# facebookresearch/r3m

Measured on AMD Instinct MI355X. Metric: encoder frames/sec (fwd+bwd) ResNet-50 224^2 bs=256/GPU, higher is better.
Workload: dtype f32

## Files before the change

r3m_amd/csrc/common.h:

```cpp
#pragma once
#include <hip/hip_runtime.h>
#include <stdint.h>
#include <stddef.h>

#ifdef R3M_PROBES
#include <cstdlib>
#define R3M_ENV_INT(name, dflt) ([]() -> int { static const int v_ = []() { const char* e_ = getenv(name); return e_ ? atoi(e_) : (dflt); }(); return v_; }())
#define R3M_PROBE(p) ((p).debug)
#else
#define R3M_ENV_INT(name, dflt) (dflt)
#define R3M_PROBE(p) 0
#endif

namespace r3m {

typedef float f32x4 __attribute__((ext_vector_type(4)));
typedef float f32x16 __attribute__((ext_vector_type(16)));

void set_last_error(const char* fmt, ...);
int  check_launch(const char* what);

#define R3M_REQUIRE(cond, ...)                  \
  do {                                          \
    if (!(cond)) {                              \
// ... 38 lines not shown
  const float* bn_scale;
  const float* bn_shift;
  const float* bn_mean;
  int N, Hi, Wi, Ci;
  int Hg, Wg;
  int Ho, Wo, Nc;
  int is;
  int os, ooy, oox;
  int M;
  int T;
  int ntaps;
  int flags;
  int simple_rows;
  int debug;
  int dtype;
  unsigned* tile_ctr;
  signed char dy[MAX_TAPS];
  signed char dx[MAX_TAPS];
  unsigned char wt[MAX_TAPS];
  int tap[MAX_TAPS];
};

struct WgradParams {
  const float* dY;
  const float* X;
  float* out;
  int N, Hi, Wi, Ci;
  int Ho, Wo, Co;
  int KH, KW, stride, pad;
  int M;
  int simple_rows;
  int dtype;
  int rows_per_split;
  int tilesN;
  int gx;
  int xcd;
  int debug;
};

int debug_occupancy(int* out4);
int launch_gather_gemm(const GatherGemmParams& p, hipStream_t s);
double gather_gemm_alg_bytes(const GatherGemmParams& p, int elem_bytes);
bool gather_gemm_fuses_affine(const GatherGemmParams& p);
int gather_gemm_grid_m(int M, int Nc);
void gg_set_tile_counters(unsigned* ctr8, int sets = 1);
int gg_set_dynamic_tiles(int on);
void gg_route_record_begin(int* out, int cap);
int gg_route_record_end();
struct WtEntry { long long w_off, wt_off; int Co, T, Ci, pad_; };
int launch_transpose_w_all(const float* params, void* wt, const WtEntry* tab, const int* tile0, int n, int tiles, int dt, hipStream_t s);
int launch_transpose_w(const float* W, float* Wt, int Co, int T, int Ci, hipStream_t s);

bool pw_gemm_eligible(const GatherGemmParams& p);
int pw_gemm_form(const GatherGemmParams& p);
int launch_pw_gemm(const GatherGemmParams& p, hipStream_t s);

enum : int {
  WG_TAPS_SIMPLE = 40,
  WG_TAPS_GATHER = 41,
  WG_ROWS        = 42,
  WG_WINDOW      = 43,
  WG16_TAPS      = 50,
  WG16_ROWS      = 51,
  WG16_ALL_TAPS  = 52,
};
struct WgradPlan {
  int route, tile, bk;
  int fast;
  int split, rows_per_split;
  int tilesN, gx;
  int lds_bytes;
  int xcd, debug;
};
WgradPlan wgrad_plan(const WgradParams& p);
int launch_wgrad(const WgradParams& p, const WgradPlan& r, hipStream_t s);
int launch_wgrad_reduce(const float* partial, float* dW, long long n, int splitK, int accumulate, hipStream_t s);
int wgrad_debug_occupancy(int* out);
bool wgrad_rowwin_eligible(const WgradParams& p);
int wgrad_rowwin_lds_bytes(int tile);
int launch_wgrad_rowwin(const WgradParams& p, const WgradPlan& r, hipStream_t s);
bool wgrad_halo_eligible(const WgradParams& p);
int wgrad_halo_lds_bytes(int W);
int launch_wgrad_bf16(const WgradParams& p, const WgradPlan& r, hipStream_t s);

int launch_gather_gemm_bf16(const GatherGemmParams& p, hipStream_t s);
bool gg16_route_builds(int route, int flags);
int gg16_route(const GatherGemmParams& p);
int launch_convert_bf16(const float* src, void* dst, long long n, hipStream_t s);
int launch_transpose_w_bf16(const float* W, void* Wt, int Co, int T, int Ci, hipStream_t s);

bool row16_eligible(const GatherGemmParams& p);
int launch_conv3x3_row_bf16(const GatherGemmParams& p, hipStream_t s);
int row16_set_mode(int mode);

#ifdef R3M_PROBES
int pw16_form(const GatherGemmParams& p);
int launch_pw16(const GatherGemmParams& p, hipStream_t s);
int pw16_set_mode(int mode);
#else
static inline int pw16_form(const GatherGemmParams&) { return 0; }
static inline int launch_pw16(const GatherGemmParams&, hipStream_t) { return 1; }
static inline int pw16_set_mode(int) { return -1; }
#endif

struct FrameSource;
int launch_stem_prep(const float* x_nchw, float* xn, int F, hipStream_t s);
// ... 117 lines not shown
```

r3m_amd/csrc/conv.hip:

```cpp
#include "common.h"
#include "conv_dev.h"
#include <utility>

namespace r3m {

__device__ __attribute__((aligned(128))) float g_zero_line[2048 + 64];


template <int EPI>
__global__ __launch_bounds__(256) void gather_gemm_glds_kernel(const GatherGemmParams p) {
  constexpr int BM = 128, BN = 128, WM = 2, WN = 2, TM = 2, TN = 2;
  constexpr int STAGE = (BM + BN) * 32;
  __shared__ __attribute__((aligned(128))) float smem[2 * STAGE];

  const int tid = threadIdx.x;
  const int lane = tid & 63;
  const int wave = tid >> 6;
  const int wm = wave / WN, wn = wave % WN;
  const int gridN = (p.Nc + BN - 1) / BN;
  const int lid = xcd_remap(blockIdx.x, gridDim.x);
  const int mt = lid / gridN, nt = lid % gridN;
  const int m0 = mt * BM, n0 = nt * BN;

  const int srow = lane >> 3;
// ... 763 lines not shown

static inline bool gg_wide(int Nc) { return (Nc % 128) == 0; }

int gather_gemm_grid_m(int M, int Nc) { return gg_wide(Nc) ? ceil_div(M, 128) : ceil_div(M, 256); }

static int gg_use_glds() {
  const int v = R3M_ENV_INT("R3M_GG_GLDS", 2);
  return v;
}

#define GG_EPI_SWITCH(LAUNCH)                                                       \
  switch (p.flags) {                                                                \
    case 0: LAUNCH(0); break;                                                       \
    case EPI_STATS: LAUNCH(EPI_STATS); break;                                       \
    case EPI_ACCUM: LAUNCH(EPI_ACCUM); break;                                       \
    case EPI_MASKED_ADD: LAUNCH(EPI_MASKED_ADD); break;                             \
    case EPI_BIAS: LAUNCH(EPI_BIAS); break;                                         \
    case EPI_RELU: LAUNCH(EPI_RELU); break;                                         \
    case EPI_BIAS | EPI_RELU: LAUNCH(EPI_BIAS | EPI_RELU); break;                   \
    case EPI_MASK_OUT: LAUNCH(EPI_MASK_OUT); break;                                 \
    case EPI_BNRED: LAUNCH(EPI_BNRED); break;                                       \
    case EPI_BNRED | EPI_MASKED_ADD: LAUNCH(EPI_BNRED | EPI_MASKED_ADD); break;     \
    default:                                                                        \
      set_last_error("gather_gemm: unsupported epilogue flag combination %d", p.flags); \
      return 1;                                                                     \
  }

double gather_gemm_alg_bytes(const GatherGemmParams& p, int elem) {
  const double in = p.simple_rows ? (double)p.M * p.Ci : (double)p.N * p.Hi * p.Wi * p.Ci;
  const double out = (double)p.M * p.Nc;
  double b = elem * (in + out + (double)p.Nc * p.ntaps * p.Ci);
  if (p.flags & EPI_ACCUM) b += elem * out;
  if (p.flags & EPI_MASKED_ADD) b += elem * out + out / 8.0;
  if (p.flags & EPI_MASK_OUT) b += elem * out;
  if (p.flags & EPI_BNRED) b += elem * out + (p.bn_bits ? out / 8.0 : 0.0) + 8.0 * bnred_partial_rows(p.M) * p.Nc;
  return b;
}

static thread_local unsigned* t_tile_ctr = nullptr;
static thread_local int t_tile_ctr_sets = 0;
static int g_dynamic_tiles = 1;
void gg_set_tile_counters(unsigned* ctr8, int sets) {
  t_tile_ctr = g_dynamic_tiles ? ctr8 : nullptr;
  t_tile_ctr_sets = t_tile_ctr ? sets : 0;
}
int gg_set_dynamic_tiles(int on) { const int old = g_dynamic_tiles; g_dynamic_tiles = on ? 1 : 0; return old; }

enum : int { GG_ROUTE_WIN = 1, GG_ROUTE_PW = 10 , GG_ROUTE_K16 = 20,
             GG_ROUTE_GLDS2 = 21, GG_ROUTE_OTHER = 22, GG_ROUTE_BF16 = 30 };
static int gg_route(const GatherGemmParams& p) {
  if (p.dtype == DT_BF16) return GG_ROUTE_BF16;
  const bool glds2 = gg_use_glds() == 2 && ((p.Ci >> 5) & 1) == 0 && p.Ci <= 2048;
  if (gg_wide(p.Nc)) {
    if (R3M_ENV_INT("R3M_GG_WIN", 1) && conv3x3_win_eligible(p, 28)) return GG_ROUTE_WIN;
    if (R3M_ENV_INT("R3M_GG_PW", 1) && pw_gemm_eligible(p)) return GG_ROUTE_PW + pw_gemm_form(p);
    const int k16_mode = R3M_ENV_INT("R3M_GG_K16", 1);
    if ((p.Ci & 31) == 0 && (k16_mode == 2 || (k16_mode == 1 && p.ntaps == 1 && p.Ci <= 256 && p.Nc >= 2 * p.Ci))) return GG_ROUTE_K16;
    return glds2 ? GG_ROUTE_GLDS2 : GG_ROUTE_OTHER;
  }
  if (R3M_ENV_INT("R3M_GG_PW", 1) && pw_gemm_eligible(p)) return GG_ROUTE_PW + pw_gemm_form(p);
  return glds2 ? GG_ROUTE_GLDS2 : GG_ROUTE_OTHER;
}

static void gg_prepare(GatherGemmParams& p) {
  for (int t = 0; t < p.ntaps; ++t)
    p.tap[t] = (int)((unsigned)(unsigned char)p.dy[t] | ((unsigned)(unsigned char)p.dx[t] << 8) | ((unsigned)p.wt[t] << 16));
  p.debug = R3M_ENV_INT("R3M_GG_DEBUG", 0);
}

bool gather_gemm_fuses_affine(const GatherGemmParams& p_in) {
  GatherGemmParams p = p_in;
  gg_prepare(p);
  if (p.dtype == DT_BF16) return (p.Nc & 7) == 0 && (p.Ci & 63) == 0 && gg16_route_builds(gg16_route(p), p.flags);
  const int r = gg_route(p);
  if (r == GG_ROUTE_WIN) return p.flags == (EPI_AFFINE | EPI_RELU) || p.flags == (EPI_AFFINE | EPI_ACCUM | EPI_RELU);
  return r > GG_ROUTE_PW && r < GG_ROUTE_K16;
}
static thread_local int* t_route_out = nullptr;
static thread_local int t_route_n = 0, t_route_cap = 0;
void gg_route_record_begin(int* out, int cap) { t_route_out = out; t_route_n = 0; t_route_cap = cap; }
int gg_route_record_end() { const int n = t_route_n; t_route_out = nullptr; t_route_n = t_route_cap = 0; return n; }
static int gg_route_record(int route) {
  if (t_route_n < t_route_cap) t_route_out[t_route_n] = route;
  ++t_route_n;
  return 0;
}

enum : int { GG_OTHER_GLDS, GG_OTHER_NARROW, GG_OTHER_REG };
static int gg_other_kernel(bool wide) {
  if (!wide) return GG_OTHER_NARROW;
#ifdef R3M_PROBES
  if (!gg_use_glds()) return GG_OTHER_REG;
#endif
  return GG_OTHER_GLDS;
}

int launch_gather_gemm(const GatherGemmParams& p_in, hipStream_t s) {
  GatherGemmParams p = p_in;
  p.tile_ctr = t_tile_ctr;
  if (t_tile_ctr && --t_tile_ctr_sets > 0) t_tile_ctr += 8;
  else { t_tile_ctr = nullptr; t_tile_ctr_sets = 0; }
  R3M_REQUIRE(p.ntaps >= 0 && p.ntaps <= MAX_TAPS, "gather_gemm: ntaps=%d", p.ntaps);
  R3M_REQUIRE(p.M > 0 && p.Nc > 0, "gather_gemm: empty problem M=%d Nc=%d", p.M, p.Nc);
  gg_prepare(p);
  if (p.dtype == DT_BF16) {
    if (t_route_out) return gg_route_record(gg16_route(p));
// ... 149 lines not shown
```

r3m_amd/csrc/conv_pw.hip:

```cpp
#include "common.h"
#include "conv_dev.h"

namespace r3m {

constexpr int PW_RSRC_FLAGS = 0x00020000;

__device__ __forceinline__ float pw_ld(const void* base, int bytes, unsigned voff, int soff) {
#if defined(__HIP_DEVICE_COMPILE__)
  return __builtin_bit_cast(float, __builtin_amdgcn_raw_buffer_load_b32(
                                       __builtin_amdgcn_make_buffer_rsrc(const_cast<void*>(base), 0, bytes, PW_RSRC_FLAGS), voff, soff, 0));
#else
  return 0.f;
#endif
}
__device__ __forceinline__ unsigned pw_ldu(const void* base, int bytes, unsigned voff, int soff) {
#if defined(__HIP_DEVICE_COMPILE__)
  return __builtin_amdgcn_raw_buffer_load_b32(__builtin_amdgcn_make_buffer_rsrc(const_cast<void*>(base), 0, bytes, PW_RSRC_FLAGS), voff, soff, 0);
#else
  return 0u;
#endif
}
typedef unsigned pw_u32x4 __attribute__((ext_vector_type(4)));
__device__ __forceinline__ f32x4 pw_ld4(const void* base, int bytes, unsigned voff, int soff) {
#if defined(__HIP_DEVICE_COMPILE__)
  return __builtin_bit_cast(f32x4, __builtin_amdgcn_raw_buffer_load_b128(
                                       __builtin_amdgcn_make_buffer_rsrc(const_cast<void*>(base), 0, bytes, PW_RSRC_FLAGS), voff, soff, 0));
#else
  return f32x4{0.f, 0.f, 0.f, 0.f};
#endif
}
#ifndef PW_ST_MOD
#define PW_ST_MOD ""
#endif
__device__ __forceinline__ void pw_st4(void* base, int bytes, unsigned voff, int soff, f32x4 v) {
#if defined(__HIP_DEVICE_COMPILE__)
  const unsigned long long a = reinterpret_cast<unsigned long long>(base);
  const pw_u32x4 rsrc = {(unsigned)a, (unsigned)(a >> 32) & 0xFFFFu, (unsigned)bytes, (unsigned)PW_RSRC_FLAGS};
  asm volatile("buffer_store_dwordx4 %0, %1, %2, %3 offen" PW_ST_MOD "\n\ts_nop 3" ::"v"(v), "v"(voff), "s"(rsrc), "s"(soff) : "memory");
#endif
}
typedef unsigned pw_u32x2 __attribute__((ext_vector_type(2)));
__device__ __forceinline__ pw_u32x2 pw_ld2(const void* base, int bytes, unsigned voff) {
#if defined(__HIP_DEVICE_COMPILE__)
  return __builtin_amdgcn_raw_buffer_load_b64(__builtin_amdgcn_make_buffer_rsrc(const_cast<void*>(base), 0, bytes, PW_RSRC_FLAGS), voff, 0, 0);
#else
  return pw_u32x2{0u, 0u};
#endif
}
__device__ __forceinline__ void pw_st(void* base, int bytes, unsigned voff, int soff, float v) {
#if defined(__HIP_DEVICE_COMPILE__)
  __builtin_amdgcn_raw_buffer_store_b32(__builtin_bit_cast(unsigned, v), __builtin_amdgcn_make_buffer_rsrc(base, 0, bytes, PW_RSRC_FLAGS), voff,
                                        soff, 0);
#endif
}

__device__ __forceinline__ const float* pw_uniform_ptr(const float* q) {
  const unsigned long long v = reinterpret_cast<unsigned long long>(q);
  const unsigned lo = __builtin_amdgcn_readfirstlane((unsigned)v), hi = __builtin_amdgcn_readfirstlane((unsigned)(v >> 32));
  return reinterpret_cast<const float*>(((unsigned long long)hi << 32) | lo);
}

template <int BM, int BN, int WM, int WN, int EPI, bool YBITS = false, bool GATHER = false, bool OSTR = false, bool BURST = false>
__global__ __launch_bounds__(WM * WN * 64, WM * WN == 4 ? 2 : 1) void pw_gemm_kernel(const GatherGemmParams p, const int tiles, const int gridN) {
  constexpr int NW = WM * WN, TN = BN / WN / 32;
  static_assert(BM / WM == 64 && (TN == 1 || TN == 2) && (NW == 4 || NW == 8), "wave tile is 64 rows x 32 TN columns");
  constexpr int STAGE = (BM + BN) * 32;
  constexpr int AJ = BM / (8 * NW), BJ = BN / (8 * NW), NP = AJ + BJ;
  static_assert(AJ >= 1 && BJ >= 1 && (NP <= 8 || BURST), "a wave stages whole DMA instructions, at most one per odd MFMA slot (burst: any number)");
  constexpr int NST = 8 * TN;
  constexpr int SR = BN >= 128 ? 128 : 256, R = BM / SR;
  static_assert(R >= 1 && WM % R == 0 && (WM / R) * 64 == SR, "wave rows nest in statistics rows");
  extern __shared__ __attribute__((aligned(128))) float smem[];

  const int tid = threadIdx.x, lane = tid & 63;
  const int wave_s = __builtin_amdgcn_readfirstlane(tid >> 6);
  const int wm = wave_s / WN, wn = wave_s % WN;
  const int W = gridDim.x;
  const int K = p.Ci, Nc = p.Nc, Kb = K * 4;
  const int lrow = lane & 31, lh = lane >> 5;

  unsigned voffA[AJ], voffB[BJ];
  const int KbB = (GATHER ? p.T : 1) * Kb;
  {
    const int srow = lane >> 3, pslot = lane & 7;
#pragma unroll
    for (int j = 0; j < AJ; ++j) {
      const int r = wave_s * (BM / NW) + j * 8 + srow;
      voffA[j] = (unsigned)(r * Kb + ((pslot ^ ((r >> 1) & 7)) << 4));
    }
#pragma unroll
    for (int j = 0; j < BJ; ++j) {
      const int r = wave_s * (BN / NW) + j * 8 + srow;
      voffB[j] = (unsigned)(r * KbB + ((pslot ^ ((r >> 1) & 7)) << 4));
    }
  }
  const float* dA = p.A;
  const float* dB = p.B;
  int dAbytes = 0, dsA = 0, dsB = 0;
  auto dma_piece = [&](auto stg_c, auto pc_c) __attribute__((always_inline)) {
    constexpr int STG = decltype(stg_c)::value, pc = decltype(pc_c)::value;
    if (R3M_PROBE(p) & 8) return;
    if constexpr (pc < AJ)
      buf_dma16_uniform(dA, dAbytes, smem + STG * STAGE + wave_s * (BM / NW) * 32 + pc * 8 * 32, voffA[pc], dsA);
    else
      buf_dma16_uniform(dB, BN * KbB, smem + STG * STAGE + BM * 32 + wave_s * (BN / NW) * 32 + (pc - AJ) * 8 * 32, voffB[pc - AJ], dsB);
  };
  auto dma_all = [&](auto stg_c) __attribute__((always_inline)) {
    static_for<NP>([&](auto pc_c) __attribute__((always_inline)) { dma_piece(stg_c, pc_c); });
  };
  unsigned poff[GATHER ? AJ : 1], iyx[GATHER ? AJ : 1];
  int tap_soffB = 0;
  auto aim_tile = [&](int tmt_, int tnt_) __attribute__((always_inline)) {
    const int tmt = __builtin_amdgcn_readfirstlane(tmt_), tnt = __builtin_amdgcn_readfirstlane(tnt_);
    dB = p.B + (long long)tnt * BN * (KbB / 4);
    if constexpr (!GATHER) {
      dA = p.A + (long long)tmt * BM * K;
      dAbytes = min(BM, p.M - tmt * BM) * Kb;
    } else {
      const int hw = p.Hg * p.Wg;
      const int m0t = tmt * BM;
      const int nf = __builtin_amdgcn_readfirstlane(m0t / hw);
      const long long frame = (long long)p.Hi * p.Wi * K;
      dA = pw_uniform_ptr(p.A + nf * frame);
      const long long rest = (long long)(p.N - nf) * frame * 4;
      dAbytes = __builtin_amdgcn_readfirstlane(rest < (long long)BUF_OOB ? (int)rest : (int)BUF_OOB);
      const int srow = lane >> 3, pslot = lane & 7;
      const int r0 = wave_s * (BM / NW) + srow;
      int m = m0t + r0;
      int n = m / hw;
      int rem = m - n * hw;
      int gy = rem / p.Wg;
      int gx = rem - gy * p.Wg;
#pragma unroll
      for (int j = 0; j < AJ; ++j) {
        const int r = r0 + j * 8;
        const int iy0 = gy * p.is, ix0 = gx * p.is;
        poff[j] = (unsigned)(((((n - nf) * p.Hi + iy0) * p.Wi + ix0) * K) * 4 + ((pslot ^ ((r >> 1) & 7)) << 4));
        iyx[j] = m < p.M ? (unsigned)((iy0 << 16) | ix0) : 0x40004000u;
        m += 8;
        gx += 8;
#pragma unroll
        for (int w = 0; w < 2; ++w) {
          const bool c = gx >= p.Wg;
          gx -= c ? p.Wg : 0;
          gy += c ? 1 : 0;
        }
#pragma unroll
        for (int w = 0; w < 2; ++w) {
          const bool c = gy >= p.Hg;
          gy -= c ? p.Hg : 0;
          n += c ? 1 : 0;
        }
      }
    }
  };
  auto set_tap = [&](int t) __attribute__((always_inline)) {
    if constexpr (GATHER) {
      const int pack = __builtin_amdgcn_readfirstlane(p.tap[t]);
      const int dy = (pack << 24) >> 24, dx = (pack << 16) >> 24, wt = pack >> 16;
      const int delta = (dy * p.Wi + dx) * Kb;
      tap_soffB = wt * Kb;
#pragma unroll
      for (int j = 0; j < AJ; ++j) {
        const unsigned iy = (iyx[j] >> 16) + (unsigned)dy, ix = (iyx[j] & 0xFFFFu) + (unsigned)dx;
        voffA[j] = (iy < (unsigned)p.Hi && ix < (unsigned)p.Wi) ? poff[j] + (unsigned)delta : BUF_OOB;
      }
    }
  };
  auto aim_step = [&](int chunk) __attribute__((always_inline)) {
    dsA = __builtin_amdgcn_readfirstlane(chunk * 128);
    dsB = __builtin_amdgcn_readfirstlane(tap_soffB + chunk * 128);
  };

  const float* fa[4];
  const float* fb[4];
  {
    const int xr = (lrow >> 1) & 7;
#pragma unroll
    for (int g = 0; g < 4; ++g) {
      const int go = ((2 * g + lh) ^ xr) * 4;
      fa[g] = smem + (wm * 64 + lrow) * 32 + go;
      fb[g] = smem + BM * 32 + (wn * TN * 32 + lrow) * 32 + go;
    }
  }
  f32x16 acc[2][TN];

  constexpr bool MADD = (EPI & EPI_MASKED_ADD) != 0, BNR = (EPI & EPI_BNRED) != 0, ACC = (EPI & EPI_ACCUM) != 0;
  constexpr bool AFF = (EPI & EPI_AFFINE) != 0, RELU = (EPI & EPI_RELU) != 0;
  static_assert(!(AFF && (BNR || MADD)) && (!RELU || AFF), "EPI_AFFINE / EPI_RELU: forward epilogues");
  constexpr bool PRE = MADD || BNR || ACC;
  static_assert(!(MADD && ACC), "one added tensor");
  constexpr int LPR = 8 * TN, RPS = 64 / LPR;
  const int srow = lane / LPR, scol = (lane % LPR) * 4;
  const unsigned vo4 = (unsigned)(((wm * 64 + srow) * Nc + wn * TN * 32 + scol) * 4);
  const int Nw = Nc >> 5;
  const unsigned vow = (unsigned)(((wm * 64 + lane) * Nw + wn * TN) * 4);
  f32x4 pg[PRE ? NST : 1], py[PRE ? NST : 1];
  typedef unsigned u32x2 __attribute__((ext_vector_type(2)));
  u32x2 pgm = {0u, 0u}, pym = {0u, 0u};
  const float* t_gb = nullptr;
  const float* t_yb = nullptr;
  const unsigned* t_gbits = nullptr;
  const unsigned* t_ybits = nullptr;
  int t_obytes = 0, t_bbytes = 0;
  static_assert(!OSTR || (GATHER && !MADD && !YBITS), "strided output rows: gather form, no mask words");
  unsigned orows[OSTR ? NST : 1];
  long long t_eo = 0;
  auto pre_tile = [&](int tmt, int tnt) __attribute__((always_inline)) {
    if constexpr (OSTR) {
      const int m0 = tmt * BM, n0 = tnt * BN;
      const int hw = p.Hg * p.Wg;
      const int nf = __builtin_amdgcn_readfirstlane(m0 / hw);
      const long long oframe = (long long)p.Ho * p.Wo * Nc;
      t_eo = nf * oframe + n0;
      const long long rest = ((long long)(p.N - nf) * oframe - n0) * 4;
      t_obytes = __builtin_amdgcn_readfirstlane(rest < (long long)BUF_OOB ? (int)rest : (int)BUF_OOB);
      const int m = m0 + wm * 64 + lane;
      const int n = m / hw;
      const int rem = m - n * hw;
      const int gy = rem / p.Wg, gx = rem - gy * p.Wg;
      const unsigned mine = m < p.M ? (unsigned)(((((n - nf) * p.Ho + gy * p.os + p.ooy) * p.Wo + gx * p.os + p.oox) * Nc) * 4) : BUF_OOB;
#pragma unroll
      for (int st = 0; st < NST; ++st)
        orows[st] = (unsigned)__builtin_amdgcn_ds_bpermute(4 * (st * RPS + srow), (int)mine) + (unsigned)((wn * TN * 32 + scol) * 4);
      if constexpr (ACC) t_gb = p.out + t_eo;
      if constexpr (BNR) t_yb = p.bn_y + t_eo;
    } else if constexpr (PRE) {
      const int m0 = tmt * BM, n0 = tnt * BN;
      const int rows_valid = min(BM, p.M - m0);
      const long long eo0 = (long long)m0 * Nc + n0;
      t_obytes = ((rows_valid - 1) * Nc + BN) * 4;
      t_bbytes = ((rows_valid - 1) * Nw + BN / 32) * 4;
      if constexpr (MADD) { t_gb = p.add0 + eo0; t_gbits = p.addbits + (eo0 >> 5); }
      if constexpr (ACC) t_gb = p.out + eo0;
      if constexpr (BNR) { t_yb = p.bn_y + eo0; t_ybits = YBITS ? p.bn_bits + (eo0 >> 5) : nullptr; }
    }
  };
  auto pre_piece = [&](auto pc_c) __attribute__((always_inline)) {
    if constexpr (PRE) {
      constexpr int pc = decltype(pc_c)::value;
      if (R3M_PROBE(p) & 16) return;
      int ncb = Nc * 4;
      asm volatile("" : "+s"(ncb));
      const int so = OSTR ? 0 : (pc * RPS) * ncb;
      const unsigned vo = OSTR ? orows[OSTR ? pc : 0] : vo4;
      if constexpr (MADD || ACC) pg[pc] = pw_ld4(t_gb, t_obytes, vo, so);
      if constexpr (BNR) py[pc] = pw_ld4(t_yb, t_obytes, vo, so);
      if constexpr (pc == 0) {
        if constexpr (MADD) {
          if constexpr (TN == 2) pgm = pw_ld2(t_gbits, t_bbytes, vow);
          else pgm[0] = pw_ldu(t_gbits, t_bbytes, vow, 0);
        }
        if constexpr (BNR && YBITS) {
          if constexpr (TN == 2) pym = pw_ld2(t_ybits, t_bbytes, vow);
          else pym[0] = pw_ldu(t_ybits, t_bbytes, vow, 0);
        }
      }
    }
  };

  auto kstep = [&](auto stgm_c, auto first_c, auto dma_c, auto pf_c, bool do_dma, bool do_pf) __attribute__((always_inline)) {
    constexpr int STG_M = decltype(stgm_c)::value, PF = decltype(pf_c)::value;
    constexpr bool FIRST = decltype(first_c)::value, DMA = decltype(dma_c)::value;
    using SD = std::integral_constant<int, STG_M ^ 1>;
    constexpr int FB = ((MADD && BNR) || (GATHER && BNR && AJ > 4)) ? 1 : 2;
    f32x4 af[FB][2], bf[FB][TN];
    auto frag_load = [&](auto g_c) __attribute__((always_inline)) {
      constexpr int g = decltype(g_c)::value;
#pragma unroll
      for (int t = 0; t < 2; ++t) af[g % FB][t] = *reinterpret_cast<const f32x4*>(fa[g] + STG_M * STAGE + t * 32 * 32);
#pragma unroll
      for (int t = 0; t < TN; ++t) bf[g % FB][t] = *reinterpret_cast<const f32x4*>(fb[g] + STG_M * STAGE + t * 32 * 32);
    };
    if constexpr (FB == 2) frag_load(std::integral_constant<int, 0>{});
    static_for<4>([&](auto g_c) __attribute__((always_inline)) {
      constexpr int g = decltype(g_c)::value;
      if constexpr (FB == 1) frag_load(g_c);
      if constexpr (FB == 2 && g < 3) frag_load(std::integral_constant<int, g + 1>{});
      const f32x4(&a)[2] = af[g % FB];
      const f32x4(&b)[TN] = bf[g % FB];
      static_for<4>([&](auto j_c) __attribute__((always_inline)) {
        constexpr int j = decltype(j_c)::value;
#pragma unroll
        for (int tm = 0; tm < 2; ++tm)
#pragma unroll
          for (int tn = 0; tn < TN; ++tn) {
            if constexpr (FIRST && g == 0 && j == 0) {
              const f32x16 z = {0.f, 0.f, 0.f, 0.f, 0.f, 0.f, 0.f, 0.f, 0.f, 0.f, 0.f, 0.f, 0.f, 0.f, 0.f, 0.f};
              acc[tm][tn] = __builtin_amdgcn_mfma_f32_32x32x2f32(a[tm][j], b[tn][j], z, 0, 0, 0);
            } else {
              acc[tm][tn] = __builtin_amdgcn_mfma_f32_32x32x2f32(a[tm][j], b[tn][j], acc[tm][tn], 0, 0, 0);
            }
          }
        if constexpr (PRE && PF != 0) {
          constexpr int slot = g * 4 + j;
// ... 9 lines not shown
          constexpr int slot = g * 4 + j;
          constexpr bool fire = (slot & 1) == 1 && (slot >> 1) < NP;
          constexpr int piece = slot >> 1;
          if constexpr (fire) {
            if (do_dma) {
              __builtin_amdgcn_sched_barrier(0);
              dma_piece(SD{}, std::integral_constant<int, piece>{});
              __builtin_amdgcn_sched_barrier(0);
            }
          }
        }
      });
    });
  };

  constexpr int CW = TN * 32;
  float* const slabs = smem + 2 * STAGE;
  float* slab = slabs + wave_s * (8 * CW);
  float* slab_w = slab + 4 * lh * CW + lrow;
  const float* slab_r = slab + srow * CW + scol;
  const int bp0 = 4 * srow;
  const bool hiw = TN == 2 && (lane & 8) != 0;
  const int nsh = (lane & 7) * 4;
  auto mask_nibble = [&](const u32x2& words, int st) __attribute__((always_inline)) -> unsigned {
    const unsigned w0 = (unsigned)__builtin_amdgcn_ds_bpermute(bp0 + st * RPS * 4, (int)words[0]);
    unsigned w = w0;
    if constexpr (TN == 2) {
      const unsigned w1 = (unsigned)__builtin_amdgcn_ds_bpermute(bp0 + st * RPS * 4, (int)words[1]);
      w = hiw ? w1 : w0;
    }
    return (w >> nsh) & 15u;
  };
  auto epilogue1 = [&](int emt, int ent) __attribute__((always_inline)) {
    const int m0 = emt * BM, n0 = ent * BN;
    if (R3M_PROBE(p) & 4) return;
    float st_s[TN], st_ss[TN];
    if ((EPI & EPI_STATS) != 0 && !(R3M_PROBE(p) & 2)) {
#pragma unroll
      for (int tn = 0; tn < TN; ++tn) {
        float s = 0.f, ss = 0.f;
#pragma unroll
        for (int tm = 0; tm < 2; ++tm)
#pragma unroll
          for (int r = 0; r < 16; ++r) {
            const float v = acc[tm][tn][r];
            s += v;
            ss = fmaf(v, v, ss);
          }
        st_s[tn] = s + __shfl_xor(s, 32);
        st_ss[tn] = ss + __shfl_xor(ss, 32);
      }
    }
    const int rows_valid = min(BM, p.M - m0);
    const long long eo0 = (long long)m0 * Nc + n0;
    const int obytes = OSTR ? t_obytes : ((rows_valid - 1) * Nc + BN) * 4;
    float* ob = p.out + (OSTR ? t_eo : eo0);
    f32x4 s1 = {0.f, 0.f, 0.f, 0.f}, s2 = s1, mu = s1, sc = s1, sh = s1;
    if constexpr (BNR) {
      const int col = n0 + wn * CW + scol;
      mu = *reinterpret_cast<const f32x4*>(p.bn_mean + col);
      if constexpr (!YBITS) {
        sc = *reinterpret_cast<const f32x4*>(p.bn_scale + col);
        sh = *reinterpret_cast<const f32x4*>(p.bn_shift + col);
      }
    }
    if constexpr (AFF) {
      const int col = n0 + wn * CW + scol;
      sc = *reinterpret_cast<const f32x4*>(p.bn_scale + col);
      sh = *reinterpret_cast<const f32x4*>(p.bn_shift + col);
    }
    static_for<8>([&](auto c_c) __attribute__((always_inline)) {
      constexpr int c = decltype(c_c)::value;
      constexpr int tm = c >> 2, q = c & 3;
#pragma unroll
      for (int tn = 0; tn < TN; ++tn)
#pragma unroll
        for (int e = 0; e < 4; ++e) slab_w[e * CW + tn * 32] = acc[tm][tn][4 * q + e];
      __builtin_amdgcn_wave_barrier();
      int ncb = Nc * 4;
      asm volatile("" : "+s"(ncb));
#pragma unroll
      for (int i = 0; i < TN; ++i) {
        const int st = c * TN + i;
        f32x4 v = *reinterpret_cast<const f32x4*>(slab_r + i * RPS * CW);
        if constexpr (AFF) {
#pragma unroll
          for (int e = 0; e < 4; ++e) v[e] = fmaf(v[e], sc[e], sh[e]);
        }
        if constexpr (ACC) v += pg[st];
        if constexpr (RELU) {
#pragma unroll
          for (int e = 0; e < 4; ++e) v[e] = fmaxf(v[e], 0.f);
        }
        if constexpr (MADD) {
          const unsigned nb = mask_nibble(pgm, st);
#pragma unroll
          for (int e = 0; e < 4; ++e) v[e] += ((nb >> e) & 1u) ? pg[st][e] : 0.f;
        }
        if (!(R3M_PROBE(p) & 1)) pw_st4(ob, obytes, OSTR ? orows[OSTR ? st : 0] : vo4, OSTR ? 0 : (st * RPS) * ncb, v);
        if constexpr (BNR) {
          const f32x4 y = py[st];
          unsigned nb = 0u;
          if constexpr (YBITS) nb = mask_nibble(pym, st);
#pragma unroll
          for (int e = 0; e < 4; ++e) {
            const bool on = YBITS ? (((nb >> e) & 1u) != 0u) : (fmaf(y[e], sc[e], sh[e]) > 0.f);
            const float gg = on ? v[e] : 0.f;
            s1[e] += gg;
            s2[e] = fmaf(gg, y[e] - mu[e], s2[e]);
          }
        }
      }
      __builtin_amdgcn_wave_barrier();
    });
    if ((EPI & EPI_STATS) != 0 && !(R3M_PROBE(p) & 2)) {
      if (lane < 32) {
#pragma unroll
        for (int tn = 0; tn < TN; ++tn) {
          slab[tn * 32 + lane] = st_s[tn];
          slab[CW + tn * 32 + lane] = st_ss[tn];
        }
      }
    }
    if constexpr (BNR) {
      const int g0 = m0 + wm * 64;
#pragma unroll
      for (int e = 0; e < 4; ++e)
#pragma unroll
        for (int o = LPR; o < 64; o <<= 1) {
          s1[e] += __shfl_xor(s1[e], o);
          s2[e] += __shfl_xor(s2[e], o);
        }
      if (lane < LPR && g0 < p.M) {
        const long long prow = g0 >> 6;
        const int col = n0 + wn * CW + scol;
        *reinterpret_cast<f32x4*>(p.stats + (prow * 2 + 0) * Nc + col) = s1;
        *reinterpret_cast<f32x4*>(p.stats + (prow * 2 + 1) * Nc + col) = s2;
      }
    }
  };
  auto epilogue2 = [&](int emt, int ent) __attribute__((always_inline)) {
    if constexpr ((EPI & EPI_STATS) != 0) {
      if (tid < R * BN) {
        const int r = tid / BN, c = tid - r * BN;
        const float* src = slabs + (c / CW) * (8 * CW) + (c % CW);
        float s = 0.f, ss = 0.f;
#pragma unroll
        for (int w = 0; w < WM / R; ++w) {
          const float* q = src + ((r * (WM / R) + w) * WN) * (8 * CW);
          s += q[0];
          ss += q[CW];
        }
        const long long srow = (long long)emt * R + r;
        if (srow * SR < p.M) {
          const int col = ent * BN + c;
          p.stats[(srow * 2 + 0) * Nc + col] = s;
          p.stats[(srow * 2 + 1) * Nc + col] = ss;
        }
      }
    }
  };

  const int hp = K >> 6;
  const int npairs = (GATHER ? p.ntaps : 1) * hp;
  using I0 = std::integral_constant<int, 0>;
  using I1 = std::integral_constant<int, 1>;
  using T_ = std::true_type;
  using F_ = std::false_type;
  using P1 = std::integral_constant<int, 1>;
  using P2 = std::integral_constant<int, 2>;
  const bool dyn = p.tile_ctr != nullptr;
  const int xq = blockIdx.x & 7;
  unsigned* ctr = dyn ? p.tile_ctr + xq : nullptr;
  int* nxt = reinterpret_cast<int*>(slabs + 2 * CW);
  const int gridM = tiles / gridN;
  auto ticket_tile = [&](int k, int& tmt, int& tnt) -> bool {
    const int kp = k / gridN;
    tnt = k - kp * gridN;
    tmt = kp * 8 + xq;
    return tmt < gridM;
  };
  int id = 0, mt = 0, nt = 0;
  bool has;
  int dm = 0, dn = 0;
  if (dyn) {
    if (tid == 0) *nxt = (int)__hip_atomic_fetch_add(ctr, 1u, __ATOMIC_RELAXED, __HIP_MEMORY_SCOPE_AGENT);
    __syncthreads();
    has = ticket_tile(__builtin_amdgcn_readfirstlane(*nxt), mt, nt);
  } else {
    id = xcd_remap(blockIdx.x, W);
    mt = id / gridN;
    nt = id - mt * gridN;
    dm = W / gridN;
    dn = W - dm * gridN;
    has = id < tiles;
  }

  bool pending = false;
  int pmt = 0, pnt = 0;
  if (has) {
    aim_tile(mt, nt);
    set_tap(0);
    aim_step(0);
    dma_all(I0{});
  }
  while (true) {
    unsigned ticket = 0u;
    if (has) {
      asm volatile("s_waitcnt vmcnt(0)" ::: "memory");
      __syncthreads();
      aim_step(1);
      dma_all(I1{});
      if (dyn && tid == 0) ticket = __hip_atomic_fetch_add(ctr, 1u, __ATOMIC_RELAXED, __HIP_MEMORY_SCOPE_AGENT);
    }
    if (pending) epilogue1(pmt, pnt);
    if (!has) break;
    pre_tile(mt, nt);
    kstep(I0{}, T_{}, F_{}, P1{}, false, npairs == 1);
    int nid = id + W;
    int nmt = mt + dm, nnt = nt + dn;
    if (nnt >= gridN) { nnt -= gridN; ++nmt; }
    bool nhas = nid < tiles;
    int ti = 0, cp = 0;
    for (int pr = 0; pr < npairs; ++pr) {
      const bool last = pr + 1 == npairs;
      if (pr > 0) {
        asm volatile("s_waitcnt vmcnt(0)" ::: "memory");
        __syncthreads();
        aim_step(2 * cp + 1);
        if constexpr (BURST) {
          dma_all(I1{});
          kstep(I0{}, F_{}, F_{}, P1{}, false, last);
        } else if (R3M_PROBE(p) & 32) {
          dma_all(I1{});
          kstep(I0{}, F_{}, F_{}, P1{}, false, last);
        } else {
          kstep(I0{}, F_{}, T_{}, P1{}, true, last);
        }
      }
      if (pr == 0 && dyn && tid == 0) *nxt = (int)ticket;
      asm volatile("s_waitcnt vmcnt(0)" ::: "memory");
      __syncthreads();
      if (pr == 0 && dyn) nhas = ticket_tile(__builtin_amdgcn_readfirstlane(*nxt), nmt, nnt);
      if (pr == 0 && pending) epilogue2(pmt, pnt);
      bool do_dma = true;
      if (last) {
        do_dma = nhas;
        if (nhas) {
          aim_tile(nmt, nnt);
          set_tap(0);
          aim_step(0);
        }
      } else if (cp + 1 == hp) {
        set_tap(ti + 1);
        aim_step(0);
      } else {
        aim_step(2 * cp + 2);
      }
      if constexpr (BURST) {
        if (do_dma) dma_all(I0{});
        kstep(I1{}, F_{}, F_{}, P2{}, false, last);
      } else if (R3M_PROBE(p) & 32) {
        if (do_dma) dma_all(I0{});
        kstep(I1{}, F_{}, F_{}, P2{}, false, last);
      } else {
        kstep(I1{}, F_{}, T_{}, P2{}, do_dma, last);
      }
      if (++cp == hp) { cp = 0; ++ti; }
    }
    pending = true;
    pmt = mt;
    pnt = nt;
    id = nid;
    mt = nmt;
    nt = nnt;
    has = nhas;
  }
  if constexpr ((EPI & EPI_STATS) != 0) {
    if (pending) {
      __syncthreads();
      epilogue2(pmt, pnt);
    }
  }
}

static int pw_cu_count() {
  static int cus[32] = {0};
  int dev = 0;
  if (hipGetDevice(&dev) != hipSuccess || dev < 0) return 256;
  const bool cached = dev < 32;
  if (cached) {
    const int c = __atomic_load_n(&cus[dev], __ATOMIC_RELAXED);
    if (c > 0) return c;
  }
  int n = 0;
  if (hipDeviceGetAttribute(&n, hipDeviceAttributeMultiprocessorCount, dev) != hipSuccess || n <= 0) n = 256;
  if (cached) __atomic_store_n(&cus[dev], n, __ATOMIC_RELAXED);
  return n;
}

static bool pw_flags_ok(const GatherGemmParams& p) {
  switch (p.flags) {
    case 0: case EPI_STATS: case EPI_ACCUM: case EPI_BNRED: return true;
    case EPI_AFFINE: case EPI_AFFINE | EPI_RELU: case EPI_AFFINE | EPI_ACCUM | EPI_RELU:
      return p.os == 1 && p.ooy == 0 && p.oox == 0 && p.Hg == p.Ho && p.Wg == p.Wo && p.bn_scale && p.bn_shift;
    case EPI_MASKED_ADD: case EPI_BNRED | EPI_MASKED_ADD: return p.addbits != nullptr;
    default: return false;
  }
}

int pw_gemm_form(const GatherGemmParams& p) {
  if (p.dtype != DT_F32) return 0;
  const bool dense_out = p.os == 1 && p.ooy == 0 && p.oox == 0 && p.Hg == p.Ho && p.Wg == p.Wo;
  if ((p.Ci & 63) || p.Ci > 2048 || (p.Nc & 63) || !pw_flags_ok(p)) return 0;
  if (dense_out && p.simple_rows && p.ntaps == 1 && p.T == 1 && p.dy[0] == 0 && p.dx[0] == 0 && p.wt[0] == 0) return 1;
  if (p.simple_rows || p.ntaps < 1 || p.ntaps > MAX_TAPS) return 0;
  if (p.Hi >= 16384 || p.Wi >= 16384 || p.Hi < 1 || p.Wi < 1 || p.Wg < 4 || p.Hg < 2) return 0;
  const long long frame = (long long)p.Hi * p.Wi * p.Ci * 4;
  const long long span = (512 / ((long long)p.Hg * p.Wg) + 2) * frame;
  if (span >= (long long)BUF_OOB || 128LL * p.T * p.Ci * 4 >= (long long)BUF_OOB) return 0;
  if (!dense_out) {
    if (p.os < 1 || p.ooy < 0 || p.oox < 0 || (p.Hg - 1) * p.os + p.ooy >= p.Ho || (p.Wg - 1) * p.os + p.oox >= p.Wo) return 0;
    if ((256 / ((long long)p.Hg * p.Wg) + 2) * (long long)p.Ho * p.Wo * p.Nc * 4 >= (long long)BUF_OOB) return 0;
    if (p.flags != 0 && p.flags != EPI_ACCUM && !(p.flags == EPI_BNRED && !p.bn_bits)) return 0;
    return 3;
  }
  if ((p.Nc & 127) == 0 && (p.flags & EPI_BNRED) && ((p.flags & EPI_MASKED_ADD) || p.bn_bits)) return 0;
  return 2;
}
bool pw_gemm_eligible(const GatherGemmParams& p) { return pw_gemm_form(p) != 0; }

static bool pw_burst(const GatherGemmParams& p) {
  const long long ktot = (long long)(p.simple_rows ? 1 : p.ntaps) * p.Ci;
  return (p.Nc & 127) != 0 && ktot >= 2LL * p.Nc &&
         (p.flags == EPI_STATS || p.flags == 0 || p.flags == (EPI_AFFINE | EPI_RELU) || (p.flags == EPI_BNRED && !p.bn_bits));
}

static bool pw_tile512() { return R3M_ENV_INT("R3M_PW_512", 1) != 0; }

template <int BM, int BN, int WM, int WN, bool GA, bool OS = false>
static int launch_pw_shape(const GatherGemmParams& p_in, hipStream_t s) {
  constexpr int NW = WM * WN, TN = BN / WN / 32;
  const int gridM = ceil_div(p_in.M, BM), gridN = p_in.Nc / BN;
  const long long tiles_ll = (long long)gridM * gridN;
  R3M_REQUIRE(tiles_ll < 0x7FFFFFFFLL, "pw_gemm: too many tiles");
  const int tiles = (int)tiles_ll;
  const int slots = (NW == 4 ? (BN == 64 ? 3 : 2) : 1) * pw_cu_count();
  const int W = tiles < slots ? tiles : slots;
  GatherGemmParams p = p_in;
  if (W < 64 || gridM < 64) p.tile_ctr = nullptr;
  constexpr int LDS = (2 * (BM + BN) * 32 + NW * 8 * TN * 32) * 4;
  static_assert(LDS <= 160 * 1024, "one CU's LDS");
  constexpr bool BURST_ONLY = BM / (8 * NW) + BN / (8 * NW) > 8;
#define LAUNCH_PW(E, YB)                                                                                                            \
  do {                                                                                                                             \
    static DynLdsOptIn oi;                                                                                                         \
    if (int e = ensure_dyn_lds(oi, reinterpret_cast<const void*>(pw_gemm_kernel<BM, BN, WM, WN, E, YB, GA, OS>), LDS, "pw_gemm")) return e; \
    hipLaunchKernelGGL((pw_gemm_kernel<BM, BN, WM, WN, E, YB, GA, OS>), dim3(W), dim3(NW * 64), LDS, s, p, tiles, gridN);               \
  } while (0)
#define LAUNCH_PW_BURST(E)                                                                                                          \
  do {                                                                                                                             \
    static DynLdsOptIn oi;                                                                                                         \
    if (int e = ensure_dyn_lds(oi, reinterpret_cast<const void*>(pw_gemm_kernel<BM, BN, WM, WN, E, false, GA, false, true>), LDS, "pw_gemm")) return e; \
    hipLaunchKernelGGL((pw_gemm_kernel<BM, BN, WM, WN, E, false, GA, false, true>), dim3(W), dim3(NW * 64), LDS, s, p, tiles, gridN);   \
  } while (0)
  const bool yb = p.bn_bits != nullptr;
  if constexpr (OS) {
    switch (p.flags) {
      case 0: LAUNCH_PW(0, false); return 0;
      case EPI_ACCUM: LAUNCH_PW(EPI_ACCUM, false); return 0;
      case EPI_BNRED: if (!yb) { LAUNCH_PW(EPI_BNRED, false); return 0; }
    }
    set_last_error("pw_gemm: form not built");
    return 1;
  } else {
  if constexpr (NW == 8) if (pw_burst(p)) {
    switch (p.flags) {
      case 0: LAUNCH_PW_BURST(0); return 0;
      case EPI_STATS: LAUNCH_PW_BURST(EPI_STATS); return 0;
      case EPI_AFFINE | EPI_RELU: LAUNCH_PW_BURST(EPI_AFFINE | EPI_RELU); return 0;
      case EPI_BNRED: LAUNCH_PW_BURST(EPI_BNRED); return 0;
    }
  }
  if constexpr (BURST_ONLY) {
    set_last_error("pw_gemm: form not built");
    return 1;
  } else
  switch (p.flags) {
    case 0: LAUNCH_PW(0, false); break;
    case EPI_STATS: LAUNCH_PW(EPI_STATS, false); break;
    case EPI_ACCUM: LAUNCH_PW(EPI_ACCUM, false); break;
    case EPI_AFFINE: LAUNCH_PW(EPI_AFFINE, false); break;
    case EPI_AFFINE | EPI_RELU: LAUNCH_PW(EPI_AFFINE | EPI_RELU, false); break;
    case EPI_AFFINE | EPI_ACCUM | EPI_RELU: LAUNCH_PW(EPI_AFFINE | EPI_ACCUM | EPI_RELU, false); break;
    case EPI_MASKED_ADD: LAUNCH_PW(EPI_MASKED_ADD, false); break;
    case EPI_BNRED:
      if (!yb) LAUNCH_PW(EPI_BNRED, false);
      else if constexpr (!(GA && NW == 4)) LAUNCH_PW(EPI_BNRED, true);
      else { set_last_error("pw_gemm: form not built"); return 1; }
      break;
    case EPI_BNRED | EPI_MASKED_ADD:
      if constexpr (!(GA && NW == 4)) {
        if (yb) LAUNCH_PW(EPI_BNRED | EPI_MASKED_ADD, true); else LAUNCH_PW(EPI_BNRED | EPI_MASKED_ADD, false);
      } else { set_last_error("pw_gemm: form not built"); return 1; }
      break;
    default: set_last_error("pw_gemm: unsupported epilogue flag combination %d", p.flags); return 1;
  }
  return 0;
  }
#undef LAUNCH_PW
#undef LAUNCH_PW_BURST
}

int launch_pw_gemm(const GatherGemmParams& p, hipStream_t s) {
  const bool wide = (p.Nc & 127) == 0;
  const int form = pw_gemm_form(p);
  if (form == 3) return wide ? launch_pw_shape<128, 128, 2, 2, true, true>(p, s) : launch_pw_shape<256, 64, 4, 2, true, true>(p, s);
  if (!wide && pw_burst(p) && pw_tile512()) return form == 2 ? launch_pw_shape<512, 64, 8, 1, true>(p, s) : launch_pw_shape<512, 64, 8, 1, false>(p, s);
  if (form == 2) return wide ? launch_pw_shape<128, 128, 2, 2, true>(p, s) : launch_pw_shape<256, 64, 4, 2, true>(p, s);
  return wide ? launch_pw_shape<128, 128, 2, 2, false>(p, s) : launch_pw_shape<256, 64, 4, 2, false>(p, s);
}

}
```

Before: 4199.

## Add frame-major tiling for small-spatial 3x3 convs in pointwise GEMM kernel

```diff
diff --git a/r3m_amd/csrc/common.h b/r3m_amd/csrc/common.h
--- a/r3m_amd/csrc/common.h
+++ b/r3m_amd/csrc/common.h
@@ -114,6 +114,7 @@
 int launch_transpose_w(const float* W, float* Wt, int Co, int T, int Ci, hipStream_t s);
 
 bool pw_gemm_eligible(const GatherGemmParams& p);
+bool pw_gemm_frame_major(const GatherGemmParams& p);
 int pw_gemm_form(const GatherGemmParams& p);
 int launch_pw_gemm(const GatherGemmParams& p, hipStream_t s);
 
diff --git a/r3m_amd/csrc/conv.hip b/r3m_amd/csrc/conv.hip
--- a/r3m_amd/csrc/conv.hip
+++ b/r3m_amd/csrc/conv.hip
@@ -839,6 +839,7 @@
   if (p.dtype == DT_BF16) return GG_ROUTE_BF16;
   const bool glds2 = gg_use_glds() == 2 && ((p.Ci >> 5) & 1) == 0 && p.Ci <= 2048;
   if (gg_wide(p.Nc)) {
+    if (R3M_ENV_INT("R3M_GG_PW", 1) && R3M_ENV_INT("R3M_PW_FM", 1) && pw_gemm_frame_major(p)) return GG_ROUTE_PW + 2;
     if (R3M_ENV_INT("R3M_GG_WIN", 1) && conv3x3_win_eligible(p, 28)) return GG_ROUTE_WIN;
     if (R3M_ENV_INT("R3M_GG_PW", 1) && pw_gemm_eligible(p)) return GG_ROUTE_PW + pw_gemm_form(p);
     const int k16_mode = R3M_ENV_INT("R3M_GG_K16", 1);
diff --git a/r3m_amd/csrc/conv_pw.hip b/r3m_amd/csrc/conv_pw.hip
--- a/r3m_amd/csrc/conv_pw.hip
+++ b/r3m_amd/csrc/conv_pw.hip
@@ -60,10 +60,11 @@
   return reinterpret_cast<const float*>(((unsigned long long)hi << 32) | lo);
 }
 
-template <int BM, int BN, int WM, int WN, int EPI, bool YBITS = false, bool GATHER = false, bool OSTR = false, bool BURST = false>
+template <int BM, int BN, int WM, int WN, int EPI, bool YBITS = false, bool GATHER = false, bool OSTR = false, bool BURST = false, bool FM = false>
 __global__ __launch_bounds__(WM * WN * 64, WM * WN == 4 ? 2 : 1) void pw_gemm_kernel(const GatherGemmParams p, const int tiles, const int gridN) {
   constexpr int NW = WM * WN, TN = BN / WN / 32;
   static_assert(BM / WM == 64 && (TN == 1 || TN == 2) && (NW == 4 || NW == 8), "wave tile is 64 rows x 32 TN columns");
+  static_assert(!FM || (GATHER && !OSTR && !BURST && !YBITS && BM == 128 && BN == 128 && !(EPI & EPI_MASKED_ADD)), "frame-major tiles: four-wave gather form");
   constexpr int STAGE = (BM + BN) * 32;
   constexpr int AJ = BM / (8 * NW), BJ = BN / (8 * NW), NP = AJ + BJ;
   static_assert(AJ >= 1 && BJ >= 1 && (NP <= 8 || BURST), "a wave stages whole DMA instructions, at most one per odd MFMA slot (burst: any number)");
@@ -86,7 +87,7 @@
 #pragma unroll
     for (int j = 0; j < AJ; ++j) {
       const int r = wave_s * (BM / NW) + j * 8 + srow;
-      voffA[j] = (unsigned)(r * Kb + ((pslot ^ ((r >> 1) & 7)) << 4));
+      voffA[j] = (unsigned)(r * (FM ? p.Hi * p.Wi * Kb : Kb) + ((pslot ^ ((r >> 1) & 7)) << 4));
     }
 #pragma unroll
     for (int j = 0; j < BJ; ++j) {
@@ -108,14 +109,38 @@
   auto dma_all = [&](auto stg_c) __attribute__((always_inline)) {
     static_for<NP>([&](auto pc_c) __attribute__((always_inline)) { dma_piece(stg_c, pc_c); });
   };
-  unsigned poff[GATHER ? AJ : 1], iyx[GATHER ? AJ : 1];
-  int tap_soffB = 0;
+  unsigned poff[GATHER && !FM ? AJ : 1], iyx[GATHER && !FM ? AJ : 1];
+  int tap_soffA = 0, tap_soffB = 0;
+  int fm_pix = 0;
+  unsigned fm_mask = 0u;
+  auto fm_decode = [&](int L, int& fb, int& pix) __attribute__((always_inline)) {
+    const int hw = p.Hg * p.Wg;
+    fb = __builtin_amdgcn_readfirstlane(L / hw);
+    pix = L - fb * hw;
+  };
   auto aim_tile = [&](int tmt_, int tnt_) __attribute__((always_inline)) {
     const int tmt = __builtin_amdgcn_readfirstlane(tmt_), tnt = __builtin_amdgcn_readfirstlane(tnt_);
     dB = p.B + (long long)tnt * BN * (KbB / 4);
     if constexpr (!GATHER) {
       dA = p.A + (long long)tmt * BM * K;
       dAbytes = min(BM, p.M - tmt * BM) * Kb;
+    } else if constexpr (FM) {
+      int fb, pix;
+      fm_decode(tmt, fb, pix);
+      const int y = __builtin_amdgcn_readfirstlane(pix / p.Wg), x = pix - y * p.Wg;
+      const long long frame = (long long)p.Hi * p.Wi * K;
+      dA = pw_uniform_ptr(p.A + (long long)fb * BM * frame);
+      const long long rest = (long long)(p.N - fb * BM) * frame * 4;
+      dAbytes = __builtin_amdgcn_readfirstlane(rest < (long long)BUF_OOB ? (int)rest : (int)BUF_OOB);
+      fm_pix = (y * p.Wi + x) * Kb;
+      unsigned m = 0u;
+#pragma unroll
+      for (int t = 0; t < 9; ++t) {
+        const int pack = p.tap[t];
+        const int dy = (pack << 24) >> 24, dx = (pack << 16) >> 24;
+        m |= ((unsigned)(y + dy) < (unsigned)p.Hi && (unsigned)(x + dx) < (unsigned)p.Wi) ? 1u << t : 0u;
+      }
+      fm_mask = (unsigned)__builtin_amdgcn_readfirstlane((int)m);
     } else {
       const int hw = p.Hg * p.Wg;
       const int m0t = tmt * BM;
@@ -155,7 +180,12 @@
     }
   };
   auto set_tap = [&](int t) __attribute__((always_inline)) {
-    if constexpr (GATHER) {
+    if constexpr (FM) {
+      const int pack = __builtin_amdgcn_readfirstlane(p.tap[t]);
+      const int dy = (pack << 24) >> 24, dx = (pack << 16) >> 24, wt = pack >> 16;
+      tap_soffA = fm_pix + (dy * p.Wi + dx) * Kb;
+      tap_soffB = wt * Kb;
+    } else if constexpr (GATHER) {
       const int pack = __builtin_amdgcn_readfirstlane(p.tap[t]);
       const int dy = (pack << 24) >> 24, dx = (pack << 16) >> 24, wt = pack >> 16;
       const int delta = (dy * p.Wi + dx) * Kb;
@@ -168,8 +198,17 @@
     }
   };
   auto aim_step = [&](int chunk) __attribute__((always_inline)) {
-    dsA = __builtin_amdgcn_readfirstlane(chunk * 128);
+    dsA = __builtin_amdgcn_readfirstlane(tap_soffA + chunk * 128);
     dsB = __builtin_amdgcn_readfirstlane(tap_soffB + chunk * 128);
+  };
+
+  auto fm_first = [&](unsigned m) __attribute__((always_inline)) -> int { return FM ? __builtin_ctz(m | 0x200u) : 0; };
+  auto fm_next = [&](unsigned m, int t) __attribute__((always_inline)) -> int { return FM ? __builtin_ctz((m & (~1u << t)) | 0x200u) : t + 1; };
+  auto fm_adv = [&](unsigned m, int& t, int& c) __attribute__((always_inline)) {
+    t = fm_next(m, t);
+    if (t >= 9) { t = fm_first(m); ++c; }
+    set_tap(t);
+    aim_step(c);
   };
 
   const float* fa[4];
@@ -192,7 +231,8 @@
   static_assert(!(MADD && ACC), "one added tensor");
   constexpr int LPR = 8 * TN, RPS = 64 / LPR;
   const int srow = lane / LPR, scol = (lane % LPR) * 4;
-  const unsigned vo4 = (unsigned)(((wm * 64 + srow) * Nc + wn * TN * 32 + scol) * 4);
+  const int orow = FM ? p.Ho * p.Wo * Nc : Nc;
+  const unsigned vo4 = (unsigned)(((wm * 64 + srow) * orow + wn * TN * 32 + scol) * 4);
   const int Nw = Nc >> 5;
   const unsigned vow = (unsigned)(((wm * 64 + lane) * Nw + wn * TN) * 4);
   f32x4 pg[PRE ? NST : 1], py[PRE ? NST : 1];
@@ -228,8 +268,13 @@
     } else if constexpr (PRE) {
       const int m0 = tmt * BM, n0 = tnt * BN;
       const int rows_valid = min(BM, p.M - m0);
-      const long long eo0 = (long long)m0 * Nc + n0;
-      t_obytes = ((rows_valid - 1) * Nc + BN) * 4;
+      long long eo0 = (long long)m0 * Nc + n0;
+      if constexpr (FM) {
+        int fb, pix;
+        fm_decode(tmt, fb, pix);
+        eo0 = ((long long)fb * BM * (p.Ho * p.Wo) + pix) * Nc + n0;
+      }
+      t_obytes = ((rows_valid - 1) * orow + BN) * 4;
       t_bbytes = ((rows_valid - 1) * Nw + BN / 32) * 4;
       if constexpr (MADD) { t_gb = p.add0 + eo0; t_gbits = p.addbits + (eo0 >> 5); }
       if constexpr (ACC) t_gb = p.out + eo0;
@@ -240,7 +285,7 @@
     if constexpr (PRE) {
       constexpr int pc = decltype(pc_c)::value;
       if (R3M_PROBE(p) & 16) return;
-      int ncb = Nc * 4;
+      int ncb = orow * 4;
       asm volatile("" : "+s"(ncb));
       const int so = OSTR ? 0 : (pc * RPS) * ncb;
       const unsigned vo = OSTR ? orows[OSTR ? pc : 0] : vo4;
@@ -356,8 +401,13 @@
       }
     }
     const int rows_valid = min(BM, p.M - m0);
-    const long long eo0 = (long long)m0 * Nc + n0;
-    const int obytes = OSTR ? t_obytes : ((rows_valid - 1) * Nc + BN) * 4;
+    long long eo0 = (long long)m0 * Nc + n0;
+    if constexpr (FM) {
+      int fb, pix;
+      fm_decode(emt, fb, pix);
+      eo0 = ((long long)fb * BM * (p.Ho * p.Wo) + pix) * Nc + n0;
+    }
+    const int obytes = OSTR ? t_obytes : ((rows_valid - 1) * orow + BN) * 4;
     float* ob = p.out + (OSTR ? t_eo : eo0);
     f32x4 s1 = {0.f, 0.f, 0.f, 0.f}, s2 = s1, mu = s1, sc = s1, sh = s1;
     if constexpr (BNR) {
@@ -381,7 +431,7 @@
 #pragma unroll
         for (int e = 0; e < 4; ++e) slab_w[e * CW + tn * 32] = acc[tm][tn][4 * q + e];
       __builtin_amdgcn_wave_barrier();
-      int ncb = Nc * 4;
+      int ncb = orow * 4;
       asm volatile("" : "+s"(ncb));
 #pragma unroll
       for (int i = 0; i < TN; ++i) {
@@ -466,7 +516,7 @@
   };
 
   const int hp = K >> 6;
-  const int npairs = (GATHER ? p.ntaps : 1) * hp;
+  const int npairs_all = (GATHER ? p.ntaps : 1) * hp;
   using I0 = std::integral_constant<int, 0>;
   using I1 = std::integral_constant<int, 1>;
   using T_ = std::true_type;
@@ -482,7 +532,9 @@
     const int kp = k / gridN;
     tnt = k - kp * gridN;
     tmt = kp * 8 + xq;
-    return tmt < gridM;
+    const bool ok = tmt < gridM;
+    if constexpr (FM) tmt = xcd_remap(tmt, gridM);
+    return ok;
   };
   int id = 0, mt = 0, nt = 0;
   bool has;
@@ -504,16 +556,19 @@
   int pmt = 0, pnt = 0;
   if (has) {
     aim_tile(mt, nt);
-    set_tap(0);
+    set_tap(fm_first(fm_mask));
     aim_step(0);
     dma_all(I0{});
   }
   while (true) {
+    const unsigned cmask = fm_mask;
+    const int npairs = FM ? __builtin_popcount(cmask) * hp : npairs_all;
+    int ti = fm_first(cmask), cp = 0, ch = 0;
     unsigned ticket = 0u;
     if (has) {
       asm volatile("s_waitcnt vmcnt(0)" ::: "memory");
       __syncthreads();
-      aim_step(1);
+      if constexpr (FM) fm_adv(cmask, ti, ch); else aim_step(1);
       dma_all(I1{});
       if (dyn && tid == 0) ticket = __hip_atomic_fetch_add(ctr, 1u, __ATOMIC_RELAXED, __HIP_MEMORY_SCOPE_AGENT);
     }
@@ -525,13 +580,12 @@
     int nmt = mt + dm, nnt = nt + dn;
     if (nnt >= gridN) { nnt -= gridN; ++nmt; }
     bool nhas = nid < tiles;
-    int ti = 0, cp = 0;
     for (int pr = 0; pr < npairs; ++pr) {
       const bool last = pr + 1 == npairs;
       if (pr > 0) {
         asm volatile("s_waitcnt vmcnt(0)" ::: "memory");
         __syncthreads();
-        aim_step(2 * cp + 1);
+        if constexpr (FM) fm_adv(cmask, ti, ch); else aim_step(2 * cp + 1);
         if constexpr (BURST) {
           dma_all(I1{});
           kstep(I0{}, F_{}, F_{}, P1{}, false, last);
@@ -552,9 +606,11 @@
         do_dma = nhas;
         if (nhas) {
           aim_tile(nmt, nnt);
-          set_tap(0);
+          set_tap(fm_first(fm_mask));
           aim_step(0);
         }
+      } else if constexpr (FM) {
+        fm_adv(cmask, ti, ch);
       } else if (cp + 1 == hp) {
         set_tap(ti + 1);
         aim_step(0);
@@ -570,7 +626,9 @@
       } else {
         kstep(I1{}, F_{}, T_{}, P2{}, do_dma, last);
       }
-      if (++cp == hp) { cp = 0; ++ti; }
+      if constexpr (!FM) {
+        if (++cp == hp) { cp = 0; ++ti; }
+      }
     }
     pending = true;
     pmt = mt;
@@ -613,8 +671,34 @@
   }
 }
 
+#ifndef R3M_PW_FM_MAX_PIXELS
+#define R3M_PW_FM_MAX_PIXELS (14 * 14)
+#endif
+constexpr int PW_FM_MAX_PIXELS = R3M_PW_FM_MAX_PIXELS;
+bool pw_gemm_frame_major(const GatherGemmParams& p) {
+  if (p.dtype != DT_F32 || p.simple_rows || p.ntaps != 9 || p.is != 1 || p.os != 1 || p.ooy != 0 || p.oox != 0) return false;
+  if (p.Hi < 1 || p.Wi < 1 || p.Hg != p.Hi || p.Wg != p.Wi || p.Ho != p.Hi || p.Wo != p.Wi) return false;
+  if ((long long)p.Hi * p.Wi > PW_FM_MAX_PIXELS || p.N < 128 || (p.N & 127) || p.M != p.N * p.Hi * p.Wi) return false;
+  if ((p.Ci & 63) || p.Ci > 2048 || (p.Nc & 127)) return false;
+  unsigned seen = 0;
+  for (int t = 0; t < 9; ++t) {
+    if (p.dy[t] < -1 || p.dy[t] > 1 || p.dx[t] < -1 || p.dx[t] > 1) return false;
+    seen |= 1u << ((p.dy[t] + 1) * 3 + (p.dx[t] + 1));
+  }
+  if (seen != 0x1ffu) return false;
+  switch (p.flags) {
+    case 0: case EPI_STATS: case EPI_ACCUM: break;
+    case EPI_BNRED: if (p.bn_bits) return false; break;
+    case EPI_AFFINE: case EPI_AFFINE | EPI_RELU: case EPI_AFFINE | EPI_ACCUM | EPI_RELU: if (!p.bn_scale || !p.bn_shift) return false; break;
+    default: return false;
+  }
+  const long long pix = (long long)p.Hi * p.Wi;
+  return 129 * pix * p.Ci * 4 < (long long)BUF_OOB && 128 * pix * p.Nc * 4 < (long long)BUF_OOB && 128LL * p.T * p.Ci * 4 < (long long)BUF_OOB;
+}
+
 int pw_gemm_form(const GatherGemmParams& p) {
   if (p.dtype != DT_F32) return 0;
+  if (pw_gemm_frame_major(p)) return 2;
   const bool dense_out = p.os == 1 && p.ooy == 0 && p.oox == 0 && p.Hg == p.Ho && p.Wg == p.Wo;
   if ((p.Ci & 63) || p.Ci > 2048 || (p.Nc & 63) || !pw_flags_ok(p)) return 0;
   if (dense_out && p.simple_rows && p.ntaps == 1 && p.T == 1 && p.dy[0] == 0 && p.dx[0] == 0 && p.wt[0] == 0) return 1;
@@ -642,7 +726,7 @@
 
 static bool pw_tile512() { return R3M_ENV_INT("R3M_PW_512", 1) != 0; }
 
-template <int BM, int BN, int WM, int WN, bool GA, bool OS = false>
+template <int BM, int BN, int WM, int WN, bool GA, bool OS = false, bool FMv = false>
 static int launch_pw_shape(const GatherGemmParams& p_in, hipStream_t s) {
   constexpr int NW = WM * WN, TN = BN / WN / 32;
   const int gridM = ceil_div(p_in.M, BM), gridN = p_in.Nc / BN;
@@ -659,8 +743,8 @@
 #define LAUNCH_PW(E, YB)                                                                                                            \
   do {                                                                                                                             \
     static DynLdsOptIn oi;                                                                                                         \
-    if (int e = ensure_dyn_lds(oi, reinterpret_cast<const void*>(pw_gemm_kernel<BM, BN, WM, WN, E, YB, GA, OS>), LDS, "pw_gemm")) return e; \
-    hipLaunchKernelGGL((pw_gemm_kernel<BM, BN, WM, WN, E, YB, GA, OS>), dim3(W), dim3(NW * 64), LDS, s, p, tiles, gridN);               \
+    if (int e = ensure_dyn_lds(oi, reinterpret_cast<const void*>(pw_gemm_kernel<BM, BN, WM, WN, E, YB, GA, OS, false, FMv>), LDS, "pw_gemm")) return e; \
+    hipLaunchKernelGGL((pw_gemm_kernel<BM, BN, WM, WN, E, YB, GA, OS, false, FMv>), dim3(W), dim3(NW * 64), LDS, s, p, tiles, gridN);               \
   } while (0)
 #define LAUNCH_PW_BURST(E)                                                                                                          \
   do {                                                                                                                             \
@@ -697,7 +781,10 @@
     case EPI_AFFINE: LAUNCH_PW(EPI_AFFINE, false); break;
     case EPI_AFFINE | EPI_RELU: LAUNCH_PW(EPI_AFFINE | EPI_RELU, false); break;
     case EPI_AFFINE | EPI_ACCUM | EPI_RELU: LAUNCH_PW(EPI_AFFINE | EPI_ACCUM | EPI_RELU, false); break;
-    case EPI_MASKED_ADD: LAUNCH_PW(EPI_MASKED_ADD, false); break;
+    case EPI_MASKED_ADD:
+      if constexpr (!FMv) LAUNCH_PW(EPI_MASKED_ADD, false);
+      else { set_last_error("pw_gemm: form not built"); return 1; }
+      break;
     case EPI_BNRED:
       if (!yb) LAUNCH_PW(EPI_BNRED, false);
       else if constexpr (!(GA && NW == 4)) LAUNCH_PW(EPI_BNRED, true);
@@ -719,6 +806,7 @@
 int launch_pw_gemm(const GatherGemmParams& p, hipStream_t s) {
   const bool wide = (p.Nc & 127) == 0;
   const int form = pw_gemm_form(p);
+  if (form == 2 && pw_gemm_frame_major(p)) return launch_pw_shape<128, 128, 2, 2, true, false, true>(p, s);
   if (form == 3) return wide ? launch_pw_shape<128, 128, 2, 2, true, true>(p, s) : launch_pw_shape<256, 64, 4, 2, true, true>(p, s);
   if (!wide && pw_burst(p) && pw_tile512()) return form == 2 ? launch_pw_shape<512, 64, 8, 1, true>(p, s) : launch_pw_shape<512, 64, 8, 1, false>(p, s);
   if (form == 2) return wide ? launch_pw_shape<128, 128, 2, 2, true>(p, s) : launch_pw_shape<256, 64, 4, 2, true>(p, s);
```

Measured after the change: 4231, median of 6. About the same (+0.8%).
